# AILab-CVC/CV-VAE

Hardware: AMD Instinct MI355X
Metric: encode+decode frames/sec (T=17, 512x512) (higher is better)
Workload: dtype bf16; 1 GPU; cfg3_sd3_T17_512: sd3 encode(x).mode() + decode(z), x=[1,3,17,512,512] per GPU; clips_per_gpu=1, hip_graphs=False, parallelism=independent clips x1 (no collective)

## Files before the change

### cvvae_amd/csrc/attention_kernel.hip

```cpp
#include <hip/hip_runtime.h>
#include <stdint.h>

#include "../../include/cvvae.h"
#include "conv_kernel.h"

namespace cvvae {

constexpr int FA_D = 512, FA_KB = 32, FA_QW = 32, FA_NW = 4;
constexpr int FA_KPITCH = FA_D * 2 + 16;
constexpr int FA_KBYTES = FA_KB * FA_KPITCH, FA_VBYTES = FA_D * FA_KB * 2;
constexpr int FA_BUF = FA_KBYTES + FA_VBYTES;

template <typename T>
__global__ __launch_bounds__(256) __attribute__((amdgpu_waves_per_eu(1, 1))) void flash_attn_d512_kernel(
    const T* __restrict__ q, const T* __restrict__ k, const T* __restrict__ vt, T* __restrict__ o, int N, long long ldvt, float scale_log2) {
  using v8 = typename Tr<T>::v8;
  __shared__ __attribute__((aligned(16))) char smem[2 * FA_BUF];
  const int tid = threadIdx.x, lane = tid & 63, wave = tid >> 6;
  const int l31 = lane & 31, hf = lane >> 5;
  const long long bt = blockIdx.y;
  const int q0 = blockIdx.x * (FA_QW * FA_NW) + wave * FA_QW;
  const int qi = q0 + l31 < N ? q0 + l31 : N - 1;
  const T* qrow = q + (bt * N + qi) * FA_D + hf * 8;
  v8 qf[FA_D / 16];
#pragma unroll
  for (int t = 0; t < FA_D / 16; ++t) qf[t] = *reinterpret_cast<const v8*>(qrow + t * 16);

  const T* kb_base = k + bt * (long long)N * FA_D;
  const T* vt_base = vt + bt * (long long)FA_D * ldvt;
  const int nkb = (N + FA_KB - 1) / FA_KB;
  typedef const __attribute__((address_space(1))) void* gptr_t;
  typedef __attribute__((address_space(3))) void* lptr_t;
  auto dma_k = [&](int kb, int buf) {
    char* kd = smem + buf * FA_BUF;
#pragma unroll
    for (int i = 0; i < 8; ++i) {
      const int key = wave * 8 + i;
      int kg = kb * FA_KB + key;
      kg = kg < N ? kg : N - 1;
      __builtin_amdgcn_global_load_lds((gptr_t)(kb_base + (long long)kg * FA_D + lane * 8), (lptr_t)(kd + key * FA_KPITCH), 16, 0, 0);
    }
  };
  const int v_r = lane >> 2;
  auto dma_v = [&](int kb, int buf) {
    char* vd = smem + buf * FA_BUF + FA_KBYTES;
#pragma unroll
    for (int j = 0; j < 8; ++j) {
      const int g = wave * 8 + j;
      const int d = 16 * g + v_r;
      const int c = (lane & 3) ^ ((d >> 2) & 3);
      __builtin_amdgcn_global_load_lds((gptr_t)(vt_base + (long long)d * ldvt + (long long)kb * FA_KB + c * 8), (lptr_t)(vd + g * 1024), 16, 0, 0);
    }
  };
  auto dma_wait = [&]() {
    asm volatile("s_waitcnt vmcnt(0)" ::: "memory");
    __syncthreads();
  };

  const int pi_key = 16 * ((l31 >> 2) & 1) + 4 * (l31 >> 3) + (l31 & 3);
  const unsigned k_off = (unsigned)(pi_key * FA_KPITCH + hf * 16);
  const unsigned v_row = (unsigned)((l31 >> 4) * 1024 + (l31 & 15) * 64);
  const unsigned v_sw = (unsigned)((l31 >> 2) & 3);
  auto scores = [&](const char* kd, int kb) -> f32x16 {
    constexpr int RING = 4, NT = FA_D / 16;
    f32x16 s0, s1;
#pragma unroll
    for (int r = 0; r < 16; ++r) s0[r] = s1[r] = 0.f;
    v8 kf[RING];
#pragma unroll
    for (int t = 0; t < RING - 1; ++t) kf[t] = *reinterpret_cast<const v8*>(kd + k_off + t * 32);
#pragma unroll
    for (int t = 0; t < NT; ++t) {
      if (t + RING - 1 < NT) kf[(t + RING - 1) % RING] = *reinterpret_cast<const v8*>(kd + k_off + (t + RING - 1) * 32);
      if (t & 1) s1 = Tr<T>::mfma(kf[t % RING], qf[t], s1);
      else s0 = Tr<T>::mfma(kf[t % RING], qf[t], s0);
      __builtin_amdgcn_sched_barrier(0);
    }
    f32x16 sc;
    const int key0 = kb * FA_KB + 16 * hf;
#pragma unroll
    for (int r = 0; r < 16; ++r) sc[r] = (key0 + r < N) ? (s0[r] + s1[r]) * scale_log2 : -1.0e30f;
    return sc;
  };

  float m_run = -1.0e30f;
  constexpr int P1B = 3;
  static_assert(P1B * FA_KBYTES <= 2 * FA_BUF, "pass-1 K ring must fit the pass-2 buffers");
  auto dma_k1 = [&](int kb) {
    char* kd = smem + (kb % P1B) * FA_KBYTES;
#pragma unroll
    for (int i = 0; i < 8; ++i) {
      const int key = wave * 8 + i;
      int kg = kb * FA_KB + key;
      kg = kg < N ? kg : N - 1;
      __builtin_amdgcn_global_load_lds((gptr_t)(kb_base + (long long)kg * FA_D + lane * 8), (lptr_t)(kd + key * FA_KPITCH), 16, 0, 0);
    }
  };
  for (int i = 0; i < P1B - 1 && i < nkb; ++i) dma_k1(i);
  for (int kb = 0; kb < nkb; ++kb) {
    if (kb + 1 < nkb) asm volatile("s_waitcnt vmcnt(8)" ::: "memory");
    else asm volatile("s_waitcnt vmcnt(0)" ::: "memory");
    __syncthreads();
    if (kb + P1B - 1 < nkb) dma_k1(kb + P1B - 1);
    const f32x16 sc = scores(smem + (kb % P1B) * FA_KBYTES, kb);
#pragma unroll
    for (int r = 0; r < 16; ++r) m_run = sc[r] > m_run ? sc[r] : m_run;
  }
  __syncthreads();
  {
    const float mo = __shfl_xor(m_run, 32, 64);
    m_run = mo > m_run ? mo : m_run;
  }

  f32x16 oacc[FA_D / 32];
#pragma unroll
  for (int b = 0; b < FA_D / 32; ++b)
#pragma unroll
    for (int r = 0; r < 16; ++r) oacc[b][r] = 0.f;
  float l_run = 0.f;
  dma_k(0, 0);
  dma_v(0, 0);
  dma_wait();
  for (int kb = 0; kb < nkb; ++kb) {
    const int cur = kb & 1;
    if (kb + 1 < nkb) {
      dma_k(kb + 1, cur ^ 1);
      dma_v(kb + 1, cur ^ 1);
    }
    const char* kd = smem + cur * FA_BUF;
    const char* vd = kd + FA_KBYTES;
    const f32x16 sc = scores(kd, kb);
    v8 pf[2];
#pragma unroll
    for (int r = 0; r < 16; ++r) {
      const float pr = __builtin_amdgcn_exp2f(sc[r] - m_run);
      pf[r >> 3][r & 7] = (T)pr;
      l_run += pr;
    }
    {
      constexpr int RING = 4, NV = 2 * (FA_D / 32);
      auto vaddr = [&](int f) { return vd + (unsigned)((f >> 1) * 2048) + v_row + (((unsigned)(2 * hf + (f & 1)) ^ v_sw) << 4); };
      v8 vf[RING];
#pragma unroll
      for (int f = 0; f < RING - 1; ++f) vf[f] = *reinterpret_cast<const v8*>(vaddr(f));
#pragma unroll
      for (int f = 0; f < NV; ++f) {
        if (f + RING - 1 < NV) vf[(f + RING - 1) % RING] = *reinterpret_cast<const v8*>(vaddr(f + RING - 1));
        oacc[f >> 1] = Tr<T>::mfma(vf[f % RING], pf[f & 1], oacc[f >> 1]);
        __builtin_amdgcn_sched_barrier(0);
      }
    }
    dma_wait();
  }
  const float l_tot = l_run + __shfl_xor(l_run, 32, 64);
  const float inv = 1.0f / l_tot;
  if (q0 + l31 < N) {
    T* orow = o + (bt * N + (q0 + l31)) * FA_D + 4 * hf;
#pragma unroll
    for (int b = 0; b < FA_D / 32; ++b)
#pragma unroll
      for (int g = 0; g < 4; ++g) {
        typename Tr<T>::v4 w;
#pragma unroll
        for (int j = 0; j < 4; ++j) w[j] = (T)(oacc[b][g * 4 + j] * inv);
        *reinterpret_cast<typename Tr<T>::v4*>(orow + b * 32 + g * 8) = w;
      }
  }
}

}

using namespace cvvae;

extern "C" int cvvae_attention_d512(int32_t dtype, const void* q, const void* k, const void* vt, void* o, int32_t batch, int32_t N,
                                    int64_t ldvt, float scale, void* stream) {
  if (!q || !k || !vt || !o || batch <= 0 || N <= 0 || ldvt < ((N + 31) / 32) * 32 || (ldvt % 8)) return CVVAE_EINVAL;
  if (dtype != CVVAE_F16 && dtype != CVVAE_BF16) return CVVAE_EUNSUPPORTED;
  const dim3 grid((unsigned)((N + 127) / 128), (unsigned)batch);
  const float sl2 = scale * 1.4426950408889634f;
  hipStream_t s = (hipStream_t)stream;
  if (dtype == CVVAE_BF16)
    hipLaunchKernelGGL(flash_attn_d512_kernel<__bf16>, grid, dim3(256), 0, s, (const __bf16*)q, (const __bf16*)k, (const __bf16*)vt, (__bf16*)o, N,
                       (long long)ldvt, sl2);
  else
    hipLaunchKernelGGL(flash_attn_d512_kernel<_Float16>, grid, dim3(256), 0, s, (const _Float16*)q, (const _Float16*)k, (const _Float16*)vt,
                       (_Float16*)o, N, (long long)ldvt, sl2);
  return (int)hipGetLastError();
}
```

Measured before the change: 246.6 frames/s.

## Replace two-pass max attention with single-pass online softmax using lazy rescaling

Drops the first pass over all K blocks that computed the exact row max, which re-read K and recomputed QK^T scores. Instead the kernel tracks a running max inside the main loop and rescales the accumulators and running sum only when a block's max exceeds the current max by more than a slack of 8 (log2 units). This halves the score MFMAs and K traffic. In exchange it adds a wave-wide vote and occasional rescale work through AGPR reads and writes, and exp2 values may reach up to 2^8, which can affect bf16 precision of P.

```diff
diff --git a/cvvae_amd/csrc/attention_kernel.hip b/cvvae_amd/csrc/attention_kernel.hip
--- a/cvvae_amd/csrc/attention_kernel.hip
+++ b/cvvae_amd/csrc/attention_kernel.hip
@@ -10,6 +10,7 @@
 constexpr int FA_KPITCH = FA_D * 2 + 16;
 constexpr int FA_KBYTES = FA_KB * FA_KPITCH, FA_VBYTES = FA_D * FA_KB * 2;
 constexpr int FA_BUF = FA_KBYTES + FA_VBYTES;
+constexpr float FA_SLACK = 8.0f;
 
 template <typename T>
 __global__ __launch_bounds__(256) __attribute__((amdgpu_waves_per_eu(1, 1))) void flash_attn_d512_kernel(
@@ -84,34 +85,6 @@
   };
 
   float m_run = -1.0e30f;
-  constexpr int P1B = 3;
-  static_assert(P1B * FA_KBYTES <= 2 * FA_BUF, "pass-1 K ring must fit the pass-2 buffers");
-  auto dma_k1 = [&](int kb) {
-    char* kd = smem + (kb % P1B) * FA_KBYTES;
-#pragma unroll
-    for (int i = 0; i < 8; ++i) {
-      const int key = wave * 8 + i;
-      int kg = kb * FA_KB + key;
-      kg = kg < N ? kg : N - 1;
-      __builtin_amdgcn_global_load_lds((gptr_t)(kb_base + (long long)kg * FA_D + lane * 8), (lptr_t)(kd + key * FA_KPITCH), 16, 0, 0);
-    }
-  };
-  for (int i = 0; i < P1B - 1 && i < nkb; ++i) dma_k1(i);
-  for (int kb = 0; kb < nkb; ++kb) {
-    if (kb + 1 < nkb) asm volatile("s_waitcnt vmcnt(8)" ::: "memory");
-    else asm volatile("s_waitcnt vmcnt(0)" ::: "memory");
-    __syncthreads();
-    if (kb + P1B - 1 < nkb) dma_k1(kb + P1B - 1);
-    const f32x16 sc = scores(smem + (kb % P1B) * FA_KBYTES, kb);
-#pragma unroll
-    for (int r = 0; r < 16; ++r) m_run = sc[r] > m_run ? sc[r] : m_run;
-  }
-  __syncthreads();
-  {
-    const float mo = __shfl_xor(m_run, 32, 64);
-    m_run = mo > m_run ? mo : m_run;
-  }
-
   f32x16 oacc[FA_D / 32];
 #pragma unroll
   for (int b = 0; b < FA_D / 32; ++b)
@@ -130,6 +103,28 @@
     const char* kd = smem + cur * FA_BUF;
     const char* vd = kd + FA_KBYTES;
     const f32x16 sc = scores(kd, kb);
+    {
+      float bm = sc[0];
+#pragma unroll
+      for (int r = 1; r < 16; ++r) bm = sc[r] > bm ? sc[r] : bm;
+      const float bo = __shfl_xor(bm, 32, 64);
+      bm = bo > bm ? bo : bm;
+      if (__any(bm > m_run + FA_SLACK)) {
+        const float m_new = bm > m_run ? bm : m_run;
+        const float alpha = __builtin_amdgcn_exp2f(m_run - m_new);
+        m_run = m_new;
+        l_run *= alpha;
+#pragma unroll
+        for (int b = 0; b < FA_D / 32; ++b)
+#pragma unroll
+          for (int r = 0; r < 16; ++r) {
+            float t;
+            asm volatile("v_accvgpr_read_b32 %1, %0\n\tv_mul_f32 %1, %1, %2\n\tv_accvgpr_write_b32 %0, %1\n\ts_nop 1"
+                         : "+a"(oacc[b][r]), "=&v"(t)
+                         : "v"(alpha));
+          }
+      }
+    }
     v8 pf[2];
 #pragma unroll
     for (int r = 0; r < 16; ++r) {
```

Result: no change. 247.7 frames/s (median of 6 runs) (+0.4%).
